# ddlau/modular_rl

Measured on NVIDIA B200. Metric: trpo_update_timesteps_per_sec, higher is better.
Workload: dtype f32

## Files before the change

### modular_rl_b200/csrc/batch_params.cu

```cuda
#include <cstdlib>
#include "common.cuh"
#include "kernels.h"
#include "comm.h"

__global__ void pack_params_kernel(NetGeom g, const float* __restrict__ theta, float* __restrict__ img,
                                   float* __restrict__ WB, int nu) {
  const int i = blockIdx.x * blockDim.x + threadIdx.x;
  const int n_wb = g.d0p * nu;
  if (i < n_wb) {
    const int k = i / nu, n = i % nu;
    const float x = (k < g.d[0] && n < g.d[1]) ? theta[g.off_flat_W[1] + k * g.d[1] + n] : 0.f;
    const float h = tf32_rna(x);
    float* base = WB + (size_t)(k >> 3) * (2 * nu * 8) + ((k & 7) >> 2) * (nu * 4) + (n >> 3) * 32 + (n & 7) * 4 + (k & 3);
    base[0] = h;
    base[nu * 8] = tf32_rna(x - h);
    return;
  }
  const int j = i - n_wb;
  if (j >= g.img_floats) return;
  float v = 0.f;
  if (j < g.bias_floats) {
    if (j >= g.off_pm_logstd) {
      const int q = j - g.off_pm_logstd;
      if (g.off_flat_logstd >= 0 && q < g.d[g.L]) v = theta[g.off_flat_logstd + q];
    } else {
      for (int l = g.L; l >= 1; --l)
        if (j >= g.off_b[l]) {
          const int q = j - g.off_b[l];
          if (q < g.d[l]) v = theta[g.off_flat_b[l] + q];
          break;
        }
    }
  } else if (j < g.bw_floats) {
    for (int l = g.L; l >= 2; --l)
      if (j >= g.off_W[l]) {
        const int q = j - g.off_W[l];
        const int row = q / g.ldw[l], col = q % g.ldw[l];
        if (col < g.d[l]) v = theta[g.off_flat_W[l] + row * g.d[l] + col];
        break;
      }
  } else {
    for (int l = g.L; l >= 2; --l)
      if (j >= g.off_WT[l]) {
        const int q = j - g.off_WT[l];
        const int row = q / g.ldt[l], col = q % g.ldt[l];
        if (col < g.d[l - 1]) v = theta[g.off_flat_W[l] + col * g.d[l] + row];
        break;
      }
  }
  img[j] = v;
}

#define RED_PX 32
#define RED_SY 8
#define RED_UN 8
#define RED_GATHER_CTAS 296
#define RED_GB 5
static_assert(RED_SY >= MRL_P2P_MAX_WORLD, "one thread row per rank in the exchange phase");
__global__ void __launch_bounds__(RED_PX * RED_SY) reduce_partials_kernel(
    NetGeom g, const float* __restrict__ part1, const float* __restrict__ partm, int n_slabs, double scale,
    const float* __restrict__ theta, double l2c2, const float* __restrict__ vlogstd_src, double vls,
    float* __restrict__ out32, double* __restrict__ out64, P2pPush push, P2pGather ga) {
  __shared__ double acc[RED_SY][RED_PX];
  const int px = threadIdx.x, sy = threadIdx.y;
  const int n_chunks = (g.P + RED_PX - 1) / RED_PX;
  for (int chunk = blockIdx.x; chunk < n_chunks; chunk += gridDim.x) {
    const int i = chunk * RED_PX + px;
    double s0 = 0.0, s1 = 0.0;
// ... 275 lines not shown
```

### modular_rl_b200/csrc/common.cuh

```cuda
#pragma once
#include <cuda_runtime.h>
#include <stdint.h>

#define MRL_TILE 64
#define MRL_LDT 68
#define MRL_MAX_LAYERS 6
#define MRL_MID_THREADS 256
#define MRL_MAX_SLAB_TILES 16

enum { MRL_HEAD_GAUSS = 0, MRL_HEAD_CAT = 1, MRL_HEAD_VALUE = 2 };
enum { MRL_ACT_TANH = 0, MRL_ACT_RELU = 1, MRL_ACT_SIGMOID = 2 };
enum { MRL_MODE_GRAD = 0, MRL_MODE_FVP = 1 };

static inline __host__ __device__ int round_up(int x, int m) { return (x + m - 1) / m * m; }

struct NetGeom {
  int L;
  int d[MRL_MAX_LAYERS + 1];
  int head, act;
  int d0p;
  int n1p;
  int ldw[MRL_MAX_LAYERS + 1];
  int ldt[MRL_MAX_LAYERS + 1];
  int off_b[MRL_MAX_LAYERS + 1];
// ... 29 lines not shown
      ".reg .pred p;\n"
      "WAIT_%=:\n"
      "mbarrier.try_wait.parity.shared::cta.b64 p, [%0], %1;\n"
      "@p bra DONE_%=;\n"
      "bra WAIT_%=;\n"
      "DONE_%=:\n"
      "}\n" ::"r"(smem_u32(bar)),
      "r"(parity)
      : "memory");
}
__device__ __forceinline__ void fence_barrier_init() {
  asm volatile("fence.mbarrier_init.release.cluster;" ::: "memory");
}
__device__ __forceinline__ void fence_proxy_async() {
  asm volatile("fence.proxy.async.shared::cta;" ::: "memory");
}
__device__ __forceinline__ void bulk_g2s(void* dst_smem, const void* src_gmem, uint32_t bytes, uint64_t* bar) {
  asm volatile("cp.async.bulk.shared::cluster.global.mbarrier::complete_tx::bytes [%0], [%1], %2, [%3];" ::"r"(
                   smem_u32(dst_smem)),
               "l"(src_gmem), "r"(bytes), "r"(smem_u32(bar))
               : "memory");
}

template <int ACT>
__device__ __forceinline__ float act_fn(float z) {
  if (ACT == MRL_ACT_TANH) return tanhf(z);
  if (ACT == MRL_ACT_RELU) return fmaxf(z, 0.f);
  return 1.f / (1.f + expf(-z));
}
template <int ACT>
__device__ __forceinline__ float dact_from_h(float h) {
  if (ACT == MRL_ACT_TANH) return 1.f - h * h;
  if (ACT == MRL_ACT_RELU) return h > 0.f ? 1.f : 0.f;
  return h * (1.f - h);
}

__device__ __forceinline__ float u_minus_log1p(float u) {
  if (fabsf(u) < 0.2f) {
    float p = 1.f / 12.f;
    p = 1.f / 11.f - u * p; p = 1.f / 10.f - u * p; p = 1.f / 9.f - u * p; p = 1.f / 8.f - u * p;
    p = 1.f / 7.f - u * p;  p = 1.f / 6.f - u * p;  p = 1.f / 5.f - u * p; p = 1.f / 4.f - u * p;
    p = 1.f / 3.f - u * p;  p = 0.5f - u * p;
    return u * u * p;
  }
  return u - log1pf(u);
}

__device__ __forceinline__ float tf32_rna(float x) {
  uint32_t u;
  asm("cvt.rna.tf32.f32 %0, %1;" : "=r"(u) : "f"(x));
  return __uint_as_float(u);
}

__device__ __forceinline__ float warp_sum(float v) {
#pragma unroll
  for (int o = 16; o > 0; o >>= 1) v += __shfl_xor_sync(0xffffffffu, v, o);
  return v;
}
__device__ __forceinline__ double warp_sum(double v) {
#pragma unroll
  for (int o = 16; o > 0; o >>= 1) v += __shfl_xor_sync(0xffffffffu, v, o);
  return v;
}
__device__ __forceinline__ double block_sum(double v, double* scratch) {
  v = warp_sum(v);
  int lane = threadIdx.x & 31, w = threadIdx.x >> 5;
  __syncthreads();
  if (lane == 0) scratch[w] = v;
  __syncthreads();
  int nw = (blockDim.x + 31) >> 5;
  double t = 0.0;
  if (w == 0) {
    t = lane < nw ? scratch[lane] : 0.0;
    t = warp_sum(t);
  }
  return t;
}

void mrl_build_geom(NetGeom* g, int n_layers, const int* dims, int head, int act, int naux);
int mrl_sm_count();
cudaError_t mrl_func_smem(const void* func, size_t bytes);
```

### modular_rl_b200/csrc/geom.cu

```cuda
#include "common.cuh"
#include <string.h>
#include <mutex>
#include <vector>

int mrl_sm_count() {
  static int cache[64] = {0};
  int dev = 0;
  if (cudaGetDevice(&dev) != cudaSuccess || dev < 0 || dev >= 64) return 148;
  if (cache[dev] == 0) {
    int sms = 0;
    if (cudaDeviceGetAttribute(&sms, cudaDevAttrMultiProcessorCount, dev) != cudaSuccess || sms <= 0) sms = 148;
    cache[dev] = sms;
  }
  return cache[dev];
}
cudaError_t mrl_func_smem(const void* func, size_t bytes) {
  struct Ent { const void* f; int dev; size_t bytes; };
  static std::vector<Ent> seen;
  static std::mutex mu;
  int dev = 0;
  cudaError_t e = cudaGetDevice(&dev);
  if (e != cudaSuccess) return e;
  std::lock_guard<std::mutex> lk(mu);
  for (Ent& en : seen)
    if (en.f == func && en.dev == dev) {
      if (bytes <= en.bytes) return cudaSuccess;
      e = cudaFuncSetAttribute(func, cudaFuncAttributeMaxDynamicSharedMemorySize, (int)bytes);
      if (e == cudaSuccess) en.bytes = bytes;
      return e;
    }
  e = cudaFuncSetAttribute(func, cudaFuncAttributeMaxDynamicSharedMemorySize, (int)bytes);
  if (e == cudaSuccess) seen.push_back({func, dev, bytes});
  return e;
}

void mrl_build_geom(NetGeom* g, int n_layers, const int* dims, int head, int act, int naux) {
  memset(g, 0, sizeof(*g));
  g->L = n_layers;
  for (int l = 0; l <= n_layers; ++l) g->d[l] = dims[l];
  g->head = head;
  g->act = act;
  g->d0p = round_up(dims[0], 8);
  g->n1p = round_up(dims[1], 8);
  int pos = 0;
  for (int l = 1; l <= n_layers; ++l) {
    g->off_flat_W[l] = pos;
    pos += dims[l - 1] * dims[l];
    g->off_flat_b[l] = pos;
    pos += dims[l];
  }
  g->off_flat_logstd = -1;
  if (head == MRL_HEAD_GAUSS) {
    g->off_flat_logstd = pos;
    pos += dims[n_layers];
  }
  g->P = pos;
  int off = 0;
  for (int l = 1; l <= n_layers; ++l) {
    g->off_b[l] = off;
    off += round_up(dims[l], 4);
  }
  g->off_pm_logstd = off;
  off += round_up(dims[n_layers], 4);
  g->bias_floats = off;
  for (int l = 2; l <= n_layers; ++l) {
    g->ldw[l] = round_up(dims[l], 4);
    g->off_W[l] = off;
    off += dims[l - 1] * g->ldw[l];
  }
  g->bw_floats = off;
  for (int l = 2; l <= n_layers; ++l) {
    g->ldt[l] = round_up(dims[l - 1], 4);
    g->off_WT[l] = off;
    off += dims[l] * g->ldt[l];
  }
  g->img_floats = off;
  int rows = 0;
  for (int l = 1; l <= n_layers; ++l) {
    g->off_act[l] = rows;
    rows += dims[l];
  }
  g->act_rows = rows;
  g->naux = naux;
  g->pmid = g->bw_floats;
}
```

### modular_rl_b200/csrc/mlp_fvp_tc.cu

```cuda
#include "common.cuh"
#include "kernels.h"
#include "tc_common.cuh"
#include <string.h>

#define FT_THREADS 768
#define FT_RSTAGES 3
#define FT_DSTAGES 3
#define FT_KSLOTS 4
#define FT_MAX_R 3
#define FT_MAX_D 6
#define FT_MAX_PASS 3
#define FT_TMEM_COLS 512

struct FtRStage {
  int l, kgs, N, acc_col, w_off, v_off;
};
struct FtDStage {
  int l, kgs, N, col0, acc_col, w_off;
};
struct FtPlan {
  int L, nR, nD;
  int Kg[MRL_MAX_LAYERS + 1], Np[MRL_MAX_LAYERS + 1];
  int vboff[MRL_MAX_LAYERS + 1];
  FtRStage rs[FT_MAX_R];
// ... 764 lines not shown
                    const float send = (lane & 4) ? val[0] : val[1];
                    const float keep = (lane & 4) ? val[1] : val[0];
                    val[0] = keep + __shfl_xor_sync(0xffffffffu, send, 4);
                  }
                  val[0] += __shfl_xor_sync(0xffffffffu, val[0], 2);
                  val[0] += __shfl_xor_sync(0xffffffffu, val[0], 1);
                  if ((lane & 3) == 0) gb1w[c0 + ((lane >> 4) & 1) * 4 + ((lane >> 3) & 1) * 2 + ((lane >> 2) & 1)] += val[0];
#pragma unroll
                  for (int i = 0; i < 8; ++i) h1c[i] = h1n[i];
                }
                tc_fence_before();
                if (tr_on) FT_TR(4, (8 << 24) | c);
              }
            }
          }
        }
        ft_dbar();
        float* part = a.partm + (size_t)slab * g.pmid;
        const int et = threadIdx.x - 384;
        for (int f = et; f < g.d[1]; f += 256) {
          float sum = 0.f;
#pragma unroll
          for (int w = 0; w < 8; ++w) sum += gb1s[w * 128 + f];
          part[g.off_b[1] + f] = sum;
        }
        for (int j = et; j < g.d[L]; j += 256) part[g.off_pm_logstd + j] = 0.f;
        ft_dbar();
        for (int f = et; f < 8 * 128; f += 256) gb1s[f] = 0.f;
        ft_dbar();
      }
    }
  }
#undef FT_FOR_TILES
  tc_fence_before();
  __syncthreads();
  if (warp == 1) {
    __syncwarp();
    tc_fence_after();
    asm volatile("tcgen05.dealloc.cta_group::1.sync.aligned.b32 %0, %1;" ::"r"(tmem_base), "r"((uint32_t)FT_TMEM_COLS));
  }
}

struct FtPackJob { int off, N, kgs, l, transposed, col0, end; };
struct FtPackJobs { FtPackJob j[FT_MAX_R + FT_MAX_D]; int n; };
__global__ void ft_pack_kernel(NetGeom g, FtPackJobs jobs, const float* __restrict__ src, float* __restrict__ dst, int total,
                               float* __restrict__ WB1, int nu) {
  const int i = blockIdx.x * blockDim.x + threadIdx.x;
  if (i >= total) {
    const int j = i - total;
    if (WB1 == nullptr || j >= g.d0p * nu) return;
    const int k = j / nu, n = j % nu;
    const float x = (k < g.d[0] && n < g.d[1]) ? src[g.off_flat_W[1] + k * g.d[1] + n] : 0.f;
    const float h = tf32_rna(x);
    float* base = WB1 + (size_t)(k >> 3) * (2 * nu * 8) + ((k & 7) >> 2) * (nu * 4) + (n >> 3) * 32 + (n & 7) * 4 + (k & 3);
    base[0] = h;
    base[nu * 8] = tf32_rna(x - h);
    return;
  }
  int q = 0, base = 0;
  while (q < jobs.n - 1 && i >= jobs.j[q].end) { base = jobs.j[q].end; ++q; }
  const FtPackJob jb = jobs.j[q];
  const int e = i - base, K = jb.kgs * 8;
  const int n = e / K, k = e % K;
  const int l = jb.l;
  float x = 0.f;
  if (!jb.transposed) {
    if (n < g.d[l] && k < g.d[l - 1]) x = src[g.off_flat_W[l] + k * g.d[l] + n];
  } else {
    if (n + jb.col0 < g.d[l - 1] && k < g.d[l]) x = src[g.off_flat_W[l] + (n + jb.col0) * g.d[l] + k];
  }
  const float h = tf32_rna(x);
  float* p = dst + jb.off + (size_t)(k >> 3) * (2 * jb.N * 8) + ((k & 7) >> 2) * (jb.N * 4) + (n >> 3) * 32 + (n & 7) * 4 + (k & 3);
  p[0] = h;
  p[jb.N * 8] = tf32_rna(x - h);
}

static bool ft_build_plan(const NetGeom& g, FtPlan* P) {
  memset(P, 0, sizeof(*P));
  const int L = g.L;
  if (L < 3 || L > 4) return false;
  if (g.head != MRL_HEAD_GAUSS && g.head != MRL_HEAD_CAT) return false;
  if (g.d[L] > 64) return false;
  P->L = L;
  int vb = 0;
  for (int l = 1; l <= L; ++l) {
    if (g.d[l] > 128) return false;
    if (l >= 2 && g.d[l] > 64) return false;
    P->Kg[l] = (g.d[l] + 7) / 8;
    P->Np[l] = round_up(g.d[l], 16);
    P->vboff[l] = vb;
    vb += round_up(g.d[l], 16) + 16;
  }
  if (vb > 512) return false;
  if (P->Np[1] != l1tc_nu(g)) return false;
  int wc = 0, vc = 0;
  P->nR = L - 1;
  for (int l = 2; l <= L; ++l) {
    FtRStage& st = P->rs[l - 2];
    st.l = l; st.kgs = P->Kg[l - 1]; st.N = P->Np[l];
    st.w_off = wc; st.v_off = vc;
    wc += st.kgs * 2 * st.N * 8;
    vc += st.kgs * 2 * st.N * 8;
    if (2 * 2 * 2 * st.N * 8 > P->rstage_floats) P->rstage_floats = 2 * 2 * 2 * st.N * 8;
  }
  int nD = 0;
  for (int l = L; l >= 2; --l) {
    P->dstage_of[l] = nD;
    const int Nout = P->Np[l - 1];
    for (int col0 = 0; col0 < Nout; col0 += 64) {
// ... 127 lines not shown
```

### modular_rl_b200/csrc/mlp_l1_tc.cu

```cuda
#include <cstdlib>
#include "common.cuh"
#include "kernels.h"
#include "tc_common.cuh"

#define TC_STAGES 12
#define TC_CGROUPS 2
#define TC_THREADS (192 + 128 * TC_CGROUPS)
#define TC_M 128

#ifdef MRL_TRACE
__device__ long long g_trace[8][512];
#define TRACE(e, u) do { if (blockIdx.x == 0 && (u) < 512) g_trace[e][u] = clock64(); } while (0)
extern "C" int mrl_debug_l1_trace(long long* out) { return cudaMemcpyFromSymbol(out, g_trace, sizeof(g_trace)) != cudaSuccess; }
#else
#define TRACE(e, u) do { } while (0)
#endif
__device__ __forceinline__ void convert_stage(unsigned char* st, int blocks, uint32_t lo_off, int lane) {
  for (int b = 0; b < blocks; ++b) {
    float4* p = reinterpret_cast<float4*>(st + (size_t)b * 4096) + lane;
    float4* pl = reinterpret_cast<float4*>(st + (size_t)b * 4096 + lo_off) + lane;
    float4 x[8];
#pragma unroll
    for (int j = 0; j < 8; ++j) x[j] = p[32 * j];
#pragma unroll
    for (int j = 0; j < 8; ++j) {
      float4 h, l;
#define MRL_SPLIT(X, H, L_)                                                   \
      H = __uint_as_float((__float_as_uint(X) + 0x1000u) & 0xffffe000u);     \
      L_ = __uint_as_float(__float_as_uint(X - H) + 0x1000u);
      MRL_SPLIT(x[j].x, h.x, l.x) MRL_SPLIT(x[j].y, h.y, l.y) MRL_SPLIT(x[j].z, h.z, l.z) MRL_SPLIT(x[j].w, h.w, l.w)
#undef MRL_SPLIT
      p[32 * j] = h;
      pl[32 * j] = l;
    }
  }
  fence_proxy_async();
}

__global__ void __launch_bounds__(TC_THREADS, 1) l1_forward_tc_kernel(const float* __restrict__ XA,
                                                                      const float* __restrict__ WB,
                                                                      float* __restrict__ Zt, int kgroups,
                                                                      int xa_kgroups, int nu, int d1, int n_mtiles,
                                                                      int n_tiles, int acc_cols, int n_acc, int tmem_cols,
                                                                      int nstages, int kps, int cgroups) {
  extern __shared__ __align__(1024) unsigned char smem_raw[];
  uint64_t* full = reinterpret_cast<uint64_t*>(smem_raw);
  uint64_t* empty = full + TC_STAGES;
  uint64_t* tfull = empty + TC_STAGES;
  uint64_t* tempty = tfull + 2;
  uint64_t* conv = tempty + 2;
  uint32_t* tmem_slot = reinterpret_cast<uint32_t*>(conv + TC_STAGES);
  unsigned char* stages = smem_raw + 512;
  const uint32_t blkA = TC_M * 8 * 4, bytesB = 2 * nu * 8 * 4;
  const uint32_t offB = kps * blkA;
  const uint32_t stage_bytes = offB + kps * bytesB;
  const int spt = (kgroups + kps - 1) / kps;
  const uint32_t a_col0 = n_acc * acc_cols;
  const int warp = threadIdx.x >> 5, lane = threadIdx.x & 31;

  if (threadIdx.x == 0) {
    for (int s = 0; s < nstages; ++s) { mbar_init(&full[s], 1); mbar_init(&empty[s], 1); mbar_init(&conv[s], 4); }
    for (int a = 0; a < 2; ++a) { mbar_init(&tfull[a], 1); mbar_init(&tempty[a], 4); }
    fence_barrier_init();
  }
  if (warp == 1) {
    asm volatile("tcgen05.alloc.cta_group::1.sync.aligned.shared::cta.b32 [%0], %1;" ::"r"(smem_u32(tmem_slot)),
                 "r"((uint32_t)tmem_cols));
    asm volatile("tcgen05.relinquish_alloc_permit.cta_group::1.sync.aligned;" ::);
  }
  tc_fence_before();
  __syncthreads();
  tc_fence_after();
  const uint32_t tmem_base = *tmem_slot;

  if (warp == 0) {
    if (lane == 0) {
      int s = 0, ph = 0, u = 0;
      for (int mt = blockIdx.x; mt < n_mtiles; mt += gridDim.x) {
        const float* a_src = XA + (size_t)mt * xa_kgroups * (TC_M * 8);
        for (int q = 0; q < spt; ++q, ++u) {
          const int kg0 = q * kps, nk = min(kps, kgroups - kg0);
          mbar_wait_guard(&empty[s], ph ^ 1);
          TRACE(0, u);
          unsigned char* st = stages + (size_t)s * stage_bytes;
          mbar_expect_tx(&full[s], nk * (blkA + bytesB));
          bulk_g2s(st, a_src + (size_t)kg0 * (TC_M * 8), nk * blkA, &full[s]);
          bulk_g2s(st + offB, WB + (size_t)kg0 * (2 * nu * 8), nk * bytesB, &full[s]);
          TRACE(1, u);
          if (++s == nstages) { s = 0; ph ^= 1; }
        }
      }
    }
  } else if (warp == 1) {
    {
      const uint32_t idesc = (1u << 4) | (2u << 7) | (2u << 10) | ((uint32_t)(nu >> 3) << 17) | ((TC_M >> 4) << 24);
      const uint32_t lboB = nu * 4 * 4;
      const uint32_t desc_hi = (uint32_t)(umma_desc(0, 0, 128) >> 32);
      const uint32_t dB0 = umma_desc_lo(smem_u32(stages) + offB, lboB);
      uint32_t tcount = 0;
      int s = 0, ph = 0, u = 0;
      bool next_ready = false;
      for (int mt = blockIdx.x; mt < n_mtiles; mt += gridDim.x, ++tcount) {
        const int acc = n_acc == 2 ? (tcount & 1) : 0;
        mbar_wait_guard(&tempty[acc], (n_acc == 2 ? ((tcount >> 1) & 1) : (tcount & 1)) ^ 1);
        tc_fence_after();
        const uint32_t d_tmem = tmem_base + acc * acc_cols;
        for (int q = 0; q < spt; ++q, ++u) {
          const int nk = min(kps, kgroups - q * kps);
          TRACE(4, u);
          if (!next_ready) mbar_wait_guard(&conv[s], ph);
          TRACE(6, u);
          tc_fence_after();
          uint32_t db = dB0 + s * (stage_bytes >> 4);
          uint32_t ta = tmem_base + a_col0 + (uint32_t)(s * kps) * 16;
          if (elect_one()) {
            for (int j = 0; j < nk; ++j) {
              umma_tf32_ts(d_tmem, ta + 8, db, desc_hi, idesc, (q | j) ? 1u : 0u);
              umma_tf32_ts(d_tmem, ta, db + (bytesB >> 5), desc_hi, idesc, 1u);
              umma_tf32_ts(d_tmem, ta, db, desc_hi, idesc, 1u);
              ta += 16;
              db += bytesB >> 4;
            }
            tc_commit(&empty[s]);
            if (q == spt - 1) tc_commit(&tfull[acc]);
          }
          __syncwarp();
          {
            const int sn = s + 1 == nstages ? 0 : s + 1;
            next_ready = mbar_probe(&conv[sn], s + 1 == nstages ? ph ^ 1 : ph);
          }
          TRACE(7, u);
          if (++s == nstages) { s = 0; ph ^= 1; }
        }
      }
    }
  } else if (warp >= 6) {
    const int quarter = warp & 3;
    const int m = quarter * 32 + lane;
    const int cgroup = (warp - 6) >> 2;
    int s = cgroup, ph = 0, u = 0;
    for (int mt = blockIdx.x; cgroup < cgroups && mt < n_mtiles; mt += gridDim.x) {
      for (int q = 0; q < spt; ++q, ++u) {
        if ((u & (cgroups - 1)) != cgroup) continue;
        const int nk = min(kps, kgroups - q * kps);
        mbar_wait_guard(&full[s], ph);
        if (warp == 6 && lane == 0) TRACE(2, u);
        const unsigned char* st = stages + (size_t)s * stage_bytes;
        uint32_t ta = tmem_base + ((uint32_t)(quarter * 32) << 16) + a_col0 + (uint32_t)(s * kps) * 16;
        for (int j = 0; j < nk; ++j) {
          const float4 x0 = *reinterpret_cast<const float4*>(st + (size_t)j * blkA + (size_t)m * 16);
          const float4 x1 = *reinterpret_cast<const float4*>(st + (size_t)j * blkA + 2048 + (size_t)m * 16);
          const float x[8] = {x0.x, x0.y, x0.z, x0.w, x1.x, x1.y, x1.z, x1.w};
          uint32_t hi[8], lo[8];
#pragma unroll
          for (int k = 0; k < 8; ++k) {
            hi[k] = (__float_as_uint(x[k]) + 0x1000u) & 0xffffe000u;
            lo[k] = __float_as_uint(x[k] - __uint_as_float(hi[k])) + 0x1000u;
          }
          tmem_st8(ta, hi);
          tmem_st8(ta + 8, lo);
          ta += 16;
        }
        asm volatile("tcgen05.wait::st.sync.aligned;" ::: "memory");
        tc_fence_before();
        __syncwarp();
        if (lane == 0) mbar_arrive(&conv[s]);
        if (warp == 6 && lane == 0) TRACE(3, u);
        s += cgroups;
        if (s >= nstages) { s -= nstages; ph ^= 1; }
      }
    }
  } else if (warp >= 2 && warp < 6) {
    const int q = warp & 3;
    uint32_t tcount = 0;
    for (int mt = blockIdx.x; mt < n_mtiles; mt += gridDim.x, ++tcount) {
      const int acc = n_acc == 2 ? (tcount & 1) : 0;
      mbar_wait_guard(&tfull[acc], n_acc == 2 ? ((tcount >> 1) & 1) : (tcount & 1));
      tc_fence_after();
      const int r = q * 32 + lane;
      const int tile = 2 * mt + (r >> 6);
      float* zt = Zt + ((size_t)tile * d1) * MRL_LDT + (r & 63);
      const uint32_t taddr = tmem_base + ((uint32_t)(q * 32) << 16) + acc * acc_cols;
      for (int c0 = 0; c0 < nu; c0 += 16) {
        uint32_t v[16];
        tmem_ld16(taddr + c0, v);
        if (tile < n_tiles) {
#pragma unroll
          for (int j = 0; j < 16; ++j)
            if (c0 + j < d1) zt[(size_t)(c0 + j) * MRL_LDT] = __uint_as_float(v[j]);
        }
      }
      tc_fence_before();
      __syncwarp();
      if (lane == 0) mbar_arrive(&tempty[acc]);
    }
  }
  tc_fence_before();
  __syncthreads();
  if (warp == 1) {
    __syncwarp();
    tc_fence_after();
    asm volatile("tcgen05.dealloc.cta_group::1.sync.aligned.b32 %0, %1;" ::"r"(tmem_base), "r"((uint32_t)tmem_cols));
  }
}

__global__ void __launch_bounds__(TC_THREADS, 1) l1_grad_tc_kernel(const float* __restrict__ XG,
                                                                   const float* __restrict__ DG,
                                                                   float* __restrict__ part1, int ftiles,
                                                                   int xg_ftiles, int nu, int d0, int n1p,
                                                                   int slab_tiles, int n_tiles, int n_slabs,
                                                                   int acc_stride, int tmem_cols, int nss, int nts,
                                                                   int dg_mn, int cgroups) {
  extern __shared__ __align__(1024) unsigned char smem_raw[];
  uint64_t* full = reinterpret_cast<uint64_t*>(smem_raw);
  uint64_t* sempty = full + TC_STAGES;
  uint64_t* conv = sempty + TC_STAGES;
  uint64_t* aempty = conv + TC_STAGES;
  uint64_t* tfull = aempty + TC_STAGES;
  uint64_t* tempty = tfull + 1;
  uint32_t* tmem_slot = reinterpret_cast<uint32_t*>(tempty + 1);
  unsigned char* stages = smem_raw + 512;
  const uint32_t blkA = TC_M * 8 * 4, bytesB = 2 * nu * 8 * 4;
  const uint32_t offB = ftiles * blkA;
  const uint32_t stage_bytes = offB + bytesB;
  const uint32_t a_col0 = ftiles * acc_stride;
  const int warp = threadIdx.x >> 5, lane = threadIdx.x & 31;

  if (threadIdx.x == 0) {
    for (int s = 0; s < nss; ++s) { mbar_init(&full[s], 1); mbar_init(&sempty[s], 1); }
    for (int s = 0; s < nts; ++s) { mbar_init(&conv[s], 4); mbar_init(&aempty[s], 1); }
    mbar_init(&tfull[0], 1);
    mbar_init(&tempty[0], 4);
    fence_barrier_init();
  }
  if (warp == 1) {
    asm volatile("tcgen05.alloc.cta_group::1.sync.aligned.shared::cta.b32 [%0], %1;" ::"r"(smem_u32(tmem_slot)),
                 "r"((uint32_t)tmem_cols));
    asm volatile("tcgen05.relinquish_alloc_permit.cta_group::1.sync.aligned;" ::);
  }
  tc_fence_before();
  __syncthreads();
  tc_fence_after();
  const uint32_t tmem_base = *tmem_slot;

  if (warp == 0) {
    if (lane == 0) {
      int s = 0, ph = 0;
      for (int slab = blockIdx.x; slab < n_slabs; slab += gridDim.x) {
        const int t0 = slab * slab_tiles, t1 = min(t0 + slab_tiles, n_tiles);
        for (int tg = t0 * 8; tg < t1 * 8; ++tg) {
          mbar_wait_guard(&sempty[s], ph ^ 1);
          unsigned char* st = stages + (size_t)s * stage_bytes;
          mbar_expect_tx(&full[s], offB + bytesB);
          bulk_g2s(st, XG + (size_t)tg * xg_ftiles * (TC_M * 8), offB, &full[s]);
          bulk_g2s(st + offB, DG + (size_t)tg * (2 * nu * 8), bytesB, &full[s]);
// ... 107 lines not shown
    asm volatile("tcgen05.dealloc.cta_group::1.sync.aligned.b32 %0, %1;" ::"r"(tmem_base), "r"((uint32_t)tmem_cols));
  }
}

template <typename T>
__global__ void pack_xa_kernel(const T* __restrict__ src, long long ld, int ncols, long long N, float* __restrict__ XA,
                               int xa_kgroups, long long rows_out) {
  const long long i = (long long)blockIdx.x * blockDim.x + threadIdx.x;
  const int quads = xa_kgroups * 2;
  if (i >= rows_out * quads) return;
  const long long t = i / quads;
  const int kq4 = (int)(i % quads);
  const int kg = kq4 >> 1, khalf = kq4 & 1;
  const long long mt = t / TC_M;
  const int m = (int)(t % TC_M);
  float x[4];
#pragma unroll
  for (int j = 0; j < 4; ++j) {
    const int c = 4 * kq4 + j;
    x[j] = (t < N && c < ncols) ? (float)src[t * ld + c] : 0.f;
  }
  float* base = XA + ((size_t)mt * xa_kgroups + kg) * (TC_M * 8) + khalf * (TC_M * 4) + (m >> 3) * 32 + (m & 7) * 4;
  *reinterpret_cast<float4*>(base) = make_float4(x[0], x[1], x[2], x[3]);
}
template <typename T>
__global__ void pack_xg_kernel(const T* __restrict__ src, long long ld, int ncols, long long N, float* __restrict__ XG,
                               int xg_ftiles, long long n_tquads) {
  const int fpad = xg_ftiles * TC_M;
  const long long i = (long long)blockIdx.x * blockDim.x + threadIdx.x;
  if (i >= n_tquads * fpad) return;
  const long long tq = i / fpad;
  const int f = (int)(i % fpad);
  float x[4];
#pragma unroll
  for (int j = 0; j < 4; ++j) {
    const long long t = tq * 4 + j;
    x[j] = (t < N && f < ncols) ? (float)src[t * ld + f] : 0.f;
  }
  const long long tg = tq >> 1;
  const int khalf = (int)(tq & 1), ft = f / TC_M, fm = f % TC_M;
  float* base = XG + ((size_t)tg * xg_ftiles + ft) * (TC_M * 8) + khalf * (TC_M * 4) + (fm >> 3) * 32 + (fm & 7) * 4;
  *reinterpret_cast<float4*>(base) = make_float4(x[0], x[1], x[2], x[3]);
}

int l1tc_nu(const NetGeom& g) { return round_up(g.d[1], 16); }
size_t l1tc_wb_floats(const NetGeom& g) { return (size_t)g.d0p * l1tc_nu(g) * 2; }
size_t l1tc_xa_floats(int xa_kgroups, long long n_mtiles) { return (size_t)n_mtiles * xa_kgroups * TC_M * 8; }

cudaError_t launch_l1_forward_tc(const NetGeom& g, const float* XA, int xa_kgroups, const float* WB, float* Zt,
                                 int n_tiles, cudaStream_t st) {
  const int nu = l1tc_nu(g);
  const int acc_cols = nu <= 32 ? 32 : (nu <= 64 ? 64 : (nu <= 128 ? 128 : 256));
  const int n_acc = acc_cols <= 128 ? 2 : 1;
  static const int kps_env = getenv("MRL_L1_KPS") ? atoi(getenv("MRL_L1_KPS")) : 0;
  static const int cg_env = getenv("MRL_L1_CGROUPS") ? atoi(getenv("MRL_L1_CGROUPS")) : 0;
  int kps = 0, nstages = 0, cgroups = 1;
  for (int pass = 0; pass < 2; ++pass) {
    kps = kps_env > 0 ? kps_env : (pass == 0 ? 4 : 3);
    const size_t sb = (size_t)kps * (TC_M * 8 * 4 + 2 * (size_t)nu * 8 * 4);
    nstages = (int)((227 * 1024 - 512) / sb);
    const int tmem_room = (512 - n_acc * acc_cols) / (kps * 16);
    if (nstages > tmem_room) nstages = tmem_room;
    if (nstages > TC_STAGES) nstages = TC_STAGES;
    cgroups = (pass == 0 && nstages >= 4) ? 2 : 1;
    if (cg_env > 0) cgroups = (cg_env >= 2 && nstages >= 2) ? 2 : 1;
    if (cgroups == 2) nstages &= ~1;
    if (cgroups == 2 || cg_env > 0 || kps_env > 0) break;
  }
  if (nstages < 2) return cudaErrorInvalidConfiguration;
  const size_t stage_bytes = (size_t)kps * (TC_M * 8 * 4 + 2 * (size_t)nu * 8 * 4);
  int tmem_cols = 32;
  while (tmem_cols < n_acc * acc_cols + nstages * kps * 16) tmem_cols *= 2;
  const size_t smem = 512 + (size_t)nstages * stage_bytes;
  {
    cudaError_t e = mrl_func_smem((const void*)l1_forward_tc_kernel, smem);
    if (e != cudaSuccess) return e;
  }
  const int sms = mrl_sm_count();
  const int n_mtiles = (n_tiles + 1) / 2;
  const int grid = n_mtiles < sms ? n_mtiles : sms;
  l1_forward_tc_kernel<<<grid, TC_THREADS, smem, st>>>(XA, WB, Zt, g.d0p / 8, xa_kgroups, nu, g.d[1], n_mtiles, n_tiles,
                                                       acc_cols, n_acc, tmem_cols, nstages, kps, cgroups);
  return cudaGetLastError();
}

cudaError_t launch_pack_xa(const void* src, int dtype, long long ld, int ncols, long long N, float* XA, int xa_kgroups,
                           long long n_mtiles, cudaStream_t st) {
  const long long rows_out = n_mtiles * TC_M;
  const long long total = rows_out * xa_kgroups * 2;
  const unsigned blocks = (unsigned)((total + 255) / 256);
  if (dtype == 1) pack_xa_kernel<double><<<blocks, 256, 0, st>>>((const double*)src, ld, ncols, N, XA, xa_kgroups, rows_out);
  else pack_xa_kernel<float><<<blocks, 256, 0, st>>>((const float*)src, ld, ncols, N, XA, xa_kgroups, rows_out);
  return cudaGetLastError();
}
size_t l1tc_xg_floats(int xg_ftiles, long long n_tiles) { return (size_t)n_tiles * 8 * xg_ftiles * TC_M * 8; }
size_t l1tc_dg_floats(const NetGeom& g, long long n_tiles) { return (size_t)n_tiles * 8 * 2 * l1tc_nu(g) * 8; }

cudaError_t launch_pack_xg(const void* src, int dtype, long long ld, int ncols, long long N, float* XG, int xg_ftiles,
                           long long n_tiles, cudaStream_t st) {
  const long long n_tquads = n_tiles * 16;
  const long long total = n_tquads * xg_ftiles * TC_M;
  const unsigned blocks = (unsigned)((total + 255) / 256);
  if (dtype == 1) pack_xg_kernel<double><<<blocks, 256, 0, st>>>((const double*)src, ld, ncols, N, XG, xg_ftiles, n_tquads);
  else pack_xg_kernel<float><<<blocks, 256, 0, st>>>((const float*)src, ld, ncols, N, XG, xg_ftiles, n_tquads);
  return cudaGetLastError();
}

static bool l1g_plan(const NetGeom& g, int* acc_stride, int* nts, int* nss, int* tmem_cols, size_t* smem) {
  const int nu = l1tc_nu(g);
  const int ftiles = (g.d[0] + TC_M - 1) / TC_M;
  *acc_stride = nu;
  *nts = (512 - ftiles * nu) / (ftiles * 16);
  if (*nts > TC_STAGES) *nts = TC_STAGES;
  const size_t stage_bytes = (size_t)ftiles * TC_M * 8 * 4 + 2 * (size_t)nu * 8 * 4;
  *nss = (int)((227 * 1024 - 512) / stage_bytes);
  if (*nss > TC_STAGES) *nss = TC_STAGES;
  *tmem_cols = 32;
  while (*tmem_cols < ftiles * nu + *nts * ftiles * 16) *tmem_cols *= 2;
  *smem = 512 + (size_t)*nss * stage_bytes;
  return nu <= 256 && *nts >= 1 && *nss >= 2 && *tmem_cols <= 512;
}

cudaError_t launch_l1_grad_tc(const NetGeom& g, const float* XG, int xg_ftiles, const float* DG, float* part1,
                              int slab_tiles, int n_tiles, int n_slabs, cudaStream_t st, int dg_mn_major) {
  const int nu = l1tc_nu(g);
  const int ftiles = (g.d[0] + TC_M - 1) / TC_M;
  int acc_stride, nts, nss, tmem_cols;
  size_t smem;
  if (!l1g_plan(g, &acc_stride, &nts, &nss, &tmem_cols, &smem)) return cudaErrorInvalidConfiguration;
  {
    cudaError_t e = mrl_func_smem((const void*)l1_grad_tc_kernel, smem);
    if (e != cudaSuccess) return e;
  }
  static const int cg_env = getenv("MRL_L1_CGROUPS") ? atoi(getenv("MRL_L1_CGROUPS")) : 0;
  int cgroups = (nts >= 2 && nss >= 4) ? 2 : 1;
// ... 15 lines not shown
```

### modular_rl_b200/csrc/tc_common.cuh

```cuda
#pragma once
#include "common.cuh"

#define TC_WATCHDOG (1u << 27)
__device__ __forceinline__ void mbar_wait_guard(uint64_t* bar, uint32_t parity) {
  uint32_t done = 0, spins = 0;
  while (true) {
    asm volatile(
        "{\n.reg .pred p;\n"
        "mbarrier.try_wait.parity.shared::cta.b64 p, [%1], %2;\n"
        "selp.u32 %0, 1, 0, p;\n}\n"
        : "=r"(done)
        : "r"(smem_u32(bar)), "r"(parity)
        : "memory");
    if (done) return;
    if (++spins > TC_WATCHDOG) __trap();
  }
}
template <int NS>
__device__ __forceinline__ void mbar_wait_ns(uint64_t* bar, uint32_t parity) {
  uint32_t done = 0, spins = 0;
  while (true) {
    asm volatile(
        "{\n.reg .pred p;\n"
        "mbarrier.try_wait.parity.shared::cta.b64 p, [%1], %2;\n"
        "selp.u32 %0, 1, 0, p;\n}\n"
        : "=r"(done)
        : "r"(smem_u32(bar)), "r"(parity)
        : "memory");
    if (done) return;
    __nanosleep(NS);
    if (++spins > (1u << 24)) __trap();
  }
}
#ifndef MRL_WAIT_NS
#define MRL_WAIT_NS 40
#endif
__device__ __forceinline__ void mbar_wait_sleep(uint64_t* bar, uint32_t parity) { mbar_wait_ns<MRL_WAIT_NS>(bar, parity); }
__device__ __forceinline__ bool elect_one() {
  uint32_t pred;
  asm volatile("{\n.reg .pred P;\nelect.sync _|P, 0xffffffff;\nselp.u32 %0, 1, 0, P;\n}\n" : "=r"(pred));
  return pred != 0;
}
__device__ __forceinline__ bool mbar_probe(uint64_t* bar, uint32_t parity) {
  uint32_t done;
  asm volatile(
      "{\n.reg .pred p;\n"
      "mbarrier.test_wait.parity.shared::cta.b64 p, [%1], %2;\n"
      "selp.u32 %0, 1, 0, p;\n}\n"
      : "=r"(done)
      : "r"(smem_u32(bar)), "r"(parity)
      : "memory");
  return done != 0;
}
__device__ __forceinline__ void mbar_arrive(uint64_t* bar) {
  asm volatile("mbarrier.arrive.shared::cta.b64 _, [%0];" ::"r"(smem_u32(bar)) : "memory");
}
__device__ __forceinline__ void tc_fence_before() { asm volatile("tcgen05.fence::before_thread_sync;" ::: "memory"); }
__device__ __forceinline__ void tc_fence_after() { asm volatile("tcgen05.fence::after_thread_sync;" ::: "memory"); }
__device__ __forceinline__ void tc_commit(uint64_t* bar) {
  asm volatile("tcgen05.commit.cta_group::1.mbarrier::arrive::one.shared::cluster.b64 [%0];" ::"r"(smem_u32(bar))
               : "memory");
}
__device__ __forceinline__ uint64_t umma_desc(uint32_t smem_addr, uint32_t lbo_bytes, uint32_t sbo_bytes) {
  return (uint64_t)((smem_addr >> 4) & 0x3FFF) | ((uint64_t)((lbo_bytes >> 4) & 0x3FFF) << 16) |
         ((uint64_t)((sbo_bytes >> 4) & 0x3FFF) << 32) | (1ull << 46);
}
__device__ __forceinline__ uint32_t umma_desc_lo(uint32_t smem_addr, uint32_t lbo_bytes) {
  return ((smem_addr >> 4) & 0x3FFF) | (((lbo_bytes >> 4) & 0x3FFF) << 16);
}
__device__ __forceinline__ void umma_tf32_lo(uint32_t tmem_d, uint32_t da_lo, uint32_t db_lo, uint32_t desc_hi,
                                             uint32_t idesc, uint32_t acc) {
  asm volatile(
      "{\n.reg .pred p;\n.reg .b64 da, db;\n"
      "setp.ne.b32 p, %5, 0;\n"
      "mov.b64 da, {%1, %3};\n"
      "mov.b64 db, {%2, %3};\n"
      "tcgen05.mma.cta_group::1.kind::tf32 [%0], da, db, %4, p;\n}\n" ::"r"(tmem_d),
      "r"(da_lo), "r"(db_lo), "r"(desc_hi), "r"(idesc), "r"(acc)
      : "memory");
}
__device__ __forceinline__ void umma_tf32_ts(uint32_t tmem_d, uint32_t tmem_a, uint32_t db_lo, uint32_t desc_hi,
                                             uint32_t idesc, uint32_t acc) {
  asm volatile(
      "{\n.reg .pred p;\n.reg .b64 db;\n"
      "setp.ne.b32 p, %5, 0;\n"
      "mov.b64 db, {%2, %3};\n"
      "tcgen05.mma.cta_group::1.kind::tf32 [%0], [%1], db, %4, p;\n}\n" ::"r"(tmem_d),
      "r"(tmem_a), "r"(db_lo), "r"(desc_hi), "r"(idesc), "r"(acc)
      : "memory");
}
__device__ __forceinline__ void tmem_st8(uint32_t taddr, const uint32_t (&r)[8]) {
  asm volatile("tcgen05.st.sync.aligned.32x32b.x8.b32 [%0], {%1, %2, %3, %4, %5, %6, %7, %8};\n" ::"r"(taddr), "r"(r[0]),
               "r"(r[1]), "r"(r[2]), "r"(r[3]), "r"(r[4]), "r"(r[5]), "r"(r[6]), "r"(r[7])
               : "memory");
}
__device__ __forceinline__ void umma_tf32(uint32_t tmem_d, uint64_t da, uint64_t db, uint32_t idesc, uint32_t acc) {
  asm volatile(
      "{\n.reg .pred p;\n"
      "setp.ne.b32 p, %4, 0;\n"
      "tcgen05.mma.cta_group::1.kind::tf32 [%0], %1, %2, %3, p;\n}\n" ::"r"(tmem_d),
      "l"(da), "l"(db), "r"(idesc), "r"(acc)
      : "memory");
}
__device__ __forceinline__ void tmem_ld16(uint32_t taddr, uint32_t (&r)[16]) {
  asm volatile(
      "tcgen05.ld.sync.aligned.32x32b.x16.b32 {%0, %1, %2, %3, %4, %5, %6, %7, %8, %9, %10, %11, %12, %13, %14, %15}, "
      "[%16];\n"
      : "=r"(r[0]), "=r"(r[1]), "=r"(r[2]), "=r"(r[3]), "=r"(r[4]), "=r"(r[5]), "=r"(r[6]), "=r"(r[7]), "=r"(r[8]),
        "=r"(r[9]), "=r"(r[10]), "=r"(r[11]), "=r"(r[12]), "=r"(r[13]), "=r"(r[14]), "=r"(r[15])
// ... 5 lines not shown
```

Measured before the change: 34.59 million.

## Convert layer-1 tensor-core forward to 2-CTA cluster MMA with split B operand

Moves the layer-1 forward GEMM from single-CTA tcgen05 MMA to cta_group::2 pair MMA, with M=256 split across a 2-CTA cluster. Each CTA now loads only half of the hi/lo weight B operand, and the WB packing layout is changed to store those halves separately. The smem stage ring and the TMEM A-operand ring are split into independent pipelines with their own barriers, and converter/epilogue warps signal the leader CTA through cluster-mapped mbarriers. This reduces per-CTA B traffic and smem footprint to allow deeper pipelining, at the cost of cluster synchronisation, a fixed kps and the removal of the environment tuning knobs.

```diff
diff --git a/modular_rl_b200/csrc/batch_params.cu b/modular_rl_b200/csrc/batch_params.cu
--- a/modular_rl_b200/csrc/batch_params.cu
+++ b/modular_rl_b200/csrc/batch_params.cu
@@ -11,9 +11,9 @@
     const int k = i / nu, n = i % nu;
     const float x = (k < g.d[0] && n < g.d[1]) ? theta[g.off_flat_W[1] + k * g.d[1] + n] : 0.f;
     const float h = tf32_rna(x);
-    float* base = WB + (size_t)(k >> 3) * (2 * nu * 8) + ((k & 7) >> 2) * (nu * 4) + (n >> 3) * 32 + (n & 7) * 4 + (k & 3);
+    float* base = WB + l1tc_wb_offset(k, n, nu, g.d0p);
     base[0] = h;
-    base[nu * 8] = tf32_rna(x - h);
+    base[nu * 4] = tf32_rna(x - h);
     return;
   }
   const int j = i - n_wb;
diff --git a/modular_rl_b200/csrc/common.cuh b/modular_rl_b200/csrc/common.cuh
--- a/modular_rl_b200/csrc/common.cuh
+++ b/modular_rl_b200/csrc/common.cuh
@@ -105,6 +105,12 @@
   return __uint_as_float(u);
 }
 
+__device__ __forceinline__ size_t l1tc_wb_offset(int k, int n, int nu, int d0p) {
+  const int h = n >= (nu >> 1), nn = n - h * (nu >> 1);
+  return (size_t)h * d0p * nu + (size_t)(k >> 3) * (nu * 8) + ((k & 7) >> 2) * (nu * 2) + (nn >> 3) * 32 + (nn & 7) * 4 +
+         (k & 3);
+}
+
 __device__ __forceinline__ float warp_sum(float v) {
 #pragma unroll
   for (int o = 16; o > 0; o >>= 1) v += __shfl_xor_sync(0xffffffffu, v, o);
@@ -133,3 +139,4 @@
 void mrl_build_geom(NetGeom* g, int n_layers, const int* dims, int head, int act, int naux);
 int mrl_sm_count();
 cudaError_t mrl_func_smem(const void* func, size_t bytes);
+cudaError_t mrl_max_clusters(const void* func, int threads, size_t smem, int* clusters);
diff --git a/modular_rl_b200/csrc/geom.cu b/modular_rl_b200/csrc/geom.cu
--- a/modular_rl_b200/csrc/geom.cu
+++ b/modular_rl_b200/csrc/geom.cu
@@ -32,6 +32,29 @@
   e = cudaFuncSetAttribute(func, cudaFuncAttributeMaxDynamicSharedMemorySize, (int)bytes);
   if (e == cudaSuccess) seen.push_back({func, dev, bytes});
   return e;
+}
+
+cudaError_t mrl_max_clusters(const void* func, int threads, size_t smem, int* clusters) {
+  struct Ent { const void* f; int dev; size_t smem; int n; };
+  static std::vector<Ent> seen;
+  static std::mutex mu;
+  int dev = 0;
+  cudaError_t e = cudaGetDevice(&dev);
+  if (e != cudaSuccess) return e;
+  std::lock_guard<std::mutex> lk(mu);
+  for (const Ent& en : seen)
+    if (en.f == func && en.dev == dev && en.smem == smem) { *clusters = en.n; return cudaSuccess; }
+  cudaLaunchConfig_t cfg = {};
+  cfg.gridDim = dim3(2 * mrl_sm_count(), 1, 1);
+  cfg.blockDim = dim3(threads, 1, 1);
+  cfg.dynamicSmemBytes = smem;
+  int n = 0;
+  e = cudaOccupancyMaxActiveClusters(&n, func, &cfg);
+  if (e != cudaSuccess) return e;
+  if (n < 1) return cudaErrorInvalidConfiguration;
+  seen.push_back({func, dev, smem, n});
+  *clusters = n;
+  return cudaSuccess;
 }
 
 void mrl_build_geom(NetGeom* g, int n_layers, const int* dims, int head, int act, int naux) {
diff --git a/modular_rl_b200/csrc/mlp_fvp_tc.cu b/modular_rl_b200/csrc/mlp_fvp_tc.cu
--- a/modular_rl_b200/csrc/mlp_fvp_tc.cu
+++ b/modular_rl_b200/csrc/mlp_fvp_tc.cu
@@ -840,9 +840,9 @@
     const int k = j / nu, n = j % nu;
     const float x = (k < g.d[0] && n < g.d[1]) ? src[g.off_flat_W[1] + k * g.d[1] + n] : 0.f;
     const float h = tf32_rna(x);
-    float* base = WB1 + (size_t)(k >> 3) * (2 * nu * 8) + ((k & 7) >> 2) * (nu * 4) + (n >> 3) * 32 + (n & 7) * 4 + (k & 3);
+    float* base = WB1 + l1tc_wb_offset(k, n, nu, g.d0p);
     base[0] = h;
-    base[nu * 8] = tf32_rna(x - h);
+    base[nu * 4] = tf32_rna(x - h);
     return;
   }
   int q = 0, base = 0;
diff --git a/modular_rl_b200/csrc/mlp_l1_tc.cu b/modular_rl_b200/csrc/mlp_l1_tc.cu
--- a/modular_rl_b200/csrc/mlp_l1_tc.cu
+++ b/modular_rl_b200/csrc/mlp_l1_tc.cu
@@ -37,70 +37,76 @@
   fence_proxy_async();
 }
 
-__global__ void __launch_bounds__(TC_THREADS, 1) l1_forward_tc_kernel(const float* __restrict__ XA,
-                                                                      const float* __restrict__ WB,
-                                                                      float* __restrict__ Zt, int kgroups,
-                                                                      int xa_kgroups, int nu, int d1, int n_mtiles,
-                                                                      int n_tiles, int acc_cols, int n_acc, int tmem_cols,
-                                                                      int nstages, int kps, int cgroups) {
+__global__ void __cluster_dims__(2, 1, 1) __launch_bounds__(TC_THREADS, 1)
+    l1_forward_tc_kernel(const float* __restrict__ XA, const float* __restrict__ WB, float* __restrict__ Zt, int kgroups,
+                         int xa_kgroups, int nu, int d1, int n_mtiles, int n_tiles, int acc_cols, int n_acc,
+                         int tmem_cols, int nss, int nts, int kps, int cgroups) {
   extern __shared__ __align__(1024) unsigned char smem_raw[];
   uint64_t* full = reinterpret_cast<uint64_t*>(smem_raw);
-  uint64_t* empty = full + TC_STAGES;
-  uint64_t* tfull = empty + TC_STAGES;
+  uint64_t* sempty = full + TC_STAGES;
+  uint64_t* aempty = sempty + TC_STAGES;
+  uint64_t* conv = aempty + TC_STAGES;
+  uint64_t* tfull = conv + TC_STAGES;
   uint64_t* tempty = tfull + 2;
-  uint64_t* conv = tempty + 2;
-  uint32_t* tmem_slot = reinterpret_cast<uint32_t*>(conv + TC_STAGES);
+  uint32_t* tmem_slot = reinterpret_cast<uint32_t*>(tempty + 2);
   unsigned char* stages = smem_raw + 512;
-  const uint32_t blkA = TC_M * 8 * 4, bytesB = 2 * nu * 8 * 4;
+  const uint32_t blkA = TC_M * 8 * 4, bytesB = nu * 8 * 4;
   const uint32_t offB = kps * blkA;
   const uint32_t stage_bytes = offB + kps * bytesB;
   const int spt = (kgroups + kps - 1) / kps;
   const uint32_t a_col0 = n_acc * acc_cols;
   const int warp = threadIdx.x >> 5, lane = threadIdx.x & 31;
+  const uint32_t rank = cluster_ctarank();
+  const int pair = blockIdx.x >> 1, npairs = gridDim.x >> 1;
+  const int n_ptiles = (n_mtiles + 1) >> 1;
 
   if (threadIdx.x == 0) {
-    for (int s = 0; s < nstages; ++s) { mbar_init(&full[s], 1); mbar_init(&empty[s], 1); mbar_init(&conv[s], 4); }
-    for (int a = 0; a < 2; ++a) { mbar_init(&tfull[a], 1); mbar_init(&tempty[a], 4); }
+    for (int s = 0; s < nss; ++s) { mbar_init(&full[s], 1); mbar_init(&sempty[s], 1); }
+    for (int a = 0; a < nts; ++a) { mbar_init(&aempty[a], 1); mbar_init(&conv[a], 8); }
+    for (int a = 0; a < 2; ++a) { mbar_init(&tfull[a], 1); mbar_init(&tempty[a], 8); }
     fence_barrier_init();
   }
   if (warp == 1) {
-    asm volatile("tcgen05.alloc.cta_group::1.sync.aligned.shared::cta.b32 [%0], %1;" ::"r"(smem_u32(tmem_slot)),
+    asm volatile("tcgen05.alloc.cta_group::2.sync.aligned.shared::cta.b32 [%0], %1;" ::"r"(smem_u32(tmem_slot)),
                  "r"((uint32_t)tmem_cols));
-    asm volatile("tcgen05.relinquish_alloc_permit.cta_group::1.sync.aligned;" ::);
+    asm volatile("tcgen05.relinquish_alloc_permit.cta_group::2.sync.aligned;" ::);
   }
   tc_fence_before();
-  __syncthreads();
+  cluster_sync();
   tc_fence_after();
   const uint32_t tmem_base = *tmem_slot;
 
   if (warp == 0) {
     if (lane == 0) {
       int s = 0, ph = 0, u = 0;
-      for (int mt = blockIdx.x; mt < n_mtiles; mt += gridDim.x) {
+      const float* b_src = WB + (size_t)rank * kgroups * (nu * 8);
+      for (int pt = pair; pt < n_ptiles; pt += npairs) {
+        const int mt = 2 * pt + (int)rank;
+        const bool has_a = mt < n_mtiles;
         const float* a_src = XA + (size_t)mt * xa_kgroups * (TC_M * 8);
         for (int q = 0; q < spt; ++q, ++u) {
           const int kg0 = q * kps, nk = min(kps, kgroups - kg0);
-          mbar_wait_guard(&empty[s], ph ^ 1);
+          mbar_wait_guard(&sempty[s], ph ^ 1);
           TRACE(0, u);
           unsigned char* st = stages + (size_t)s * stage_bytes;
-          mbar_expect_tx(&full[s], nk * (blkA + bytesB));
-          bulk_g2s(st, a_src + (size_t)kg0 * (TC_M * 8), nk * blkA, &full[s]);
-          bulk_g2s(st + offB, WB + (size_t)kg0 * (2 * nu * 8), nk * bytesB, &full[s]);
+          mbar_expect_tx(&full[s], nk * ((has_a ? blkA : 0u) + bytesB));
+          if (has_a) bulk_g2s(st, a_src + (size_t)kg0 * (TC_M * 8), nk * blkA, &full[s]);
+          bulk_g2s(st + offB, b_src + (size_t)kg0 * (nu * 8), nk * bytesB, &full[s]);
           TRACE(1, u);
-          if (++s == nstages) { s = 0; ph ^= 1; }
+          if (++s == nss) { s = 0; ph ^= 1; }
         }
       }
     }
   } else if (warp == 1) {
-    {
-      const uint32_t idesc = (1u << 4) | (2u << 7) | (2u << 10) | ((uint32_t)(nu >> 3) << 17) | ((TC_M >> 4) << 24);
-      const uint32_t lboB = nu * 4 * 4;
+    if (rank == 0) {
+      const uint32_t idesc = (1u << 4) | (2u << 7) | (2u << 10) | ((uint32_t)(nu >> 3) << 17) | ((2 * TC_M >> 4) << 24);
+      const uint32_t lboB = nu * 8;
       const uint32_t desc_hi = (uint32_t)(umma_desc(0, 0, 128) >> 32);
       const uint32_t dB0 = umma_desc_lo(smem_u32(stages) + offB, lboB);
       uint32_t tcount = 0;
-      int s = 0, ph = 0, u = 0;
+      int s = 0, a = 0, aph = 0, u = 0;
       bool next_ready = false;
-      for (int mt = blockIdx.x; mt < n_mtiles; mt += gridDim.x, ++tcount) {
+      for (int pt = pair; pt < n_ptiles; pt += npairs, ++tcount) {
         const int acc = n_acc == 2 ? (tcount & 1) : 0;
         mbar_wait_guard(&tempty[acc], (n_acc == 2 ? ((tcount >> 1) & 1) : (tcount & 1)) ^ 1);
         tc_fence_after();
@@ -108,29 +114,31 @@
         for (int q = 0; q < spt; ++q, ++u) {
           const int nk = min(kps, kgroups - q * kps);
           TRACE(4, u);
-          if (!next_ready) mbar_wait_guard(&conv[s], ph);
+          if (!next_ready) mbar_wait_guard(&conv[a], aph);
           TRACE(6, u);
           tc_fence_after();
           uint32_t db = dB0 + s * (stage_bytes >> 4);
-          uint32_t ta = tmem_base + a_col0 + (uint32_t)(s * kps) * 16;
+          uint32_t ta = tmem_base + a_col0 + (uint32_t)(a * kps) * 16;
           if (elect_one()) {
             for (int j = 0; j < nk; ++j) {
-              umma_tf32_ts(d_tmem, ta + 8, db, desc_hi, idesc, (q | j) ? 1u : 0u);
-              umma_tf32_ts(d_tmem, ta, db + (bytesB >> 5), desc_hi, idesc, 1u);
-              umma_tf32_ts(d_tmem, ta, db, desc_hi, idesc, 1u);
+              umma_tf32_ts_pair(d_tmem, ta + 8, db, desc_hi, idesc, (q | j) ? 1u : 0u);
+              umma_tf32_ts_pair(d_tmem, ta, db + (bytesB >> 5), desc_hi, idesc, 1u);
+              umma_tf32_ts_pair(d_tmem, ta, db, desc_hi, idesc, 1u);
               ta += 16;
               db += bytesB >> 4;
             }
-            tc_commit(&empty[s]);
-            if (q == spt - 1) tc_commit(&tfull[acc]);
+            tc_commit_pair(&sempty[s]);
+            tc_commit_pair(&aempty[a]);
+            if (q == spt - 1) tc_commit_pair(&tfull[acc]);
           }
           __syncwarp();
           {
-            const int sn = s + 1 == nstages ? 0 : s + 1;
-            next_ready = mbar_probe(&conv[sn], s + 1 == nstages ? ph ^ 1 : ph);
+            const int an = a + 1 == nts ? 0 : a + 1;
+            next_ready = mbar_probe(&conv[an], a + 1 == nts ? aph ^ 1 : aph);
           }
           TRACE(7, u);
-          if (++s == nstages) { s = 0; ph ^= 1; }
+          if (++s == nss) s = 0;
+          if (++a == nts) { a = 0; aph ^= 1; }
         }
       }
     }
@@ -138,16 +146,19 @@
     const int quarter = warp & 3;
     const int m = quarter * 32 + lane;
     const int cgroup = (warp - 6) >> 2;
-    int s = cgroup, ph = 0, u = 0;
-    for (int mt = blockIdx.x; cgroup < cgroups && mt < n_mtiles; mt += gridDim.x) {
+    int s = cgroup, ph = 0, a = cgroup, aph = 0, u = 0;
+    for (int pt = pair; cgroup < cgroups && pt < n_ptiles; pt += npairs) {
+      const bool has_a = 2 * pt + (int)rank < n_mtiles;
       for (int q = 0; q < spt; ++q, ++u) {
         if ((u & (cgroups - 1)) != cgroup) continue;
         const int nk = min(kps, kgroups - q * kps);
         mbar_wait_guard(&full[s], ph);
+        mbar_wait_guard(&aempty[a], aph ^ 1);
+        tc_fence_after();
         if (warp == 6 && lane == 0) TRACE(2, u);
         const unsigned char* st = stages + (size_t)s * stage_bytes;
-        uint32_t ta = tmem_base + ((uint32_t)(quarter * 32) << 16) + a_col0 + (uint32_t)(s * kps) * 16;
-        for (int j = 0; j < nk; ++j) {
+        uint32_t ta = tmem_base + ((uint32_t)(quarter * 32) << 16) + a_col0 + (uint32_t)(a * kps) * 16;
+        for (int j = 0; has_a && j < nk; ++j) {
           const float4 x0 = *reinterpret_cast<const float4*>(st + (size_t)j * blkA + (size_t)m * 16);
           const float4 x1 = *reinterpret_cast<const float4*>(st + (size_t)j * blkA + 2048 + (size_t)m * 16);
           const float x[8] = {x0.x, x0.y, x0.z, x0.w, x1.x, x1.y, x1.z, x1.w};
@@ -164,21 +175,23 @@
         asm volatile("tcgen05.wait::st.sync.aligned;" ::: "memory");
         tc_fence_before();
         __syncwarp();
-        if (lane == 0) mbar_arrive(&conv[s]);
+        if (lane == 0) mbar_arrive_cluster(&conv[a], 0);
         if (warp == 6 && lane == 0) TRACE(3, u);
         s += cgroups;
-        if (s >= nstages) { s -= nstages; ph ^= 1; }
+        if (s >= nss) { s -= nss; ph ^= 1; }
+        a += cgroups;
+        if (a >= nts) { a -= nts; aph ^= 1; }
       }
     }
   } else if (warp >= 2 && warp < 6) {
     const int q = warp & 3;
     uint32_t tcount = 0;
-    for (int mt = blockIdx.x; mt < n_mtiles; mt += gridDim.x, ++tcount) {
+    for (int pt = pair; pt < n_ptiles; pt += npairs, ++tcount) {
       const int acc = n_acc == 2 ? (tcount & 1) : 0;
       mbar_wait_guard(&tfull[acc], n_acc == 2 ? ((tcount >> 1) & 1) : (tcount & 1));
       tc_fence_after();
       const int r = q * 32 + lane;
-      const int tile = 2 * mt + (r >> 6);
+      const int tile = 2 * (2 * pt + (int)rank) + (r >> 6);
       float* zt = Zt + ((size_t)tile * d1) * MRL_LDT + (r & 63);
       const uint32_t taddr = tmem_base + ((uint32_t)(q * 32) << 16) + acc * acc_cols;
       for (int c0 = 0; c0 < nu; c0 += 16) {
@@ -192,15 +205,15 @@
       }
       tc_fence_before();
       __syncwarp();
-      if (lane == 0) mbar_arrive(&tempty[acc]);
+      if (lane == 0) mbar_arrive_cluster(&tempty[acc], 0);
     }
   }
   tc_fence_before();
-  __syncthreads();
+  cluster_sync();
   if (warp == 1) {
     __syncwarp();
     tc_fence_after();
-    asm volatile("tcgen05.dealloc.cta_group::1.sync.aligned.b32 %0, %1;" ::"r"(tmem_base), "r"((uint32_t)tmem_cols));
+    asm volatile("tcgen05.dealloc.cta_group::2.sync.aligned.b32 %0, %1;" ::"r"(tmem_base), "r"((uint32_t)tmem_cols));
   }
 }
 
@@ -414,35 +427,32 @@
   const int nu = l1tc_nu(g);
   const int acc_cols = nu <= 32 ? 32 : (nu <= 64 ? 64 : (nu <= 128 ? 128 : 256));
   const int n_acc = acc_cols <= 128 ? 2 : 1;
-  static const int kps_env = getenv("MRL_L1_KPS") ? atoi(getenv("MRL_L1_KPS")) : 0;
-  static const int cg_env = getenv("MRL_L1_CGROUPS") ? atoi(getenv("MRL_L1_CGROUPS")) : 0;
-  int kps = 0, nstages = 0, cgroups = 1;
-  for (int pass = 0; pass < 2; ++pass) {
-    kps = kps_env > 0 ? kps_env : (pass == 0 ? 4 : 3);
-    const size_t sb = (size_t)kps * (TC_M * 8 * 4 + 2 * (size_t)nu * 8 * 4);
-    nstages = (int)((227 * 1024 - 512) / sb);
-    const int tmem_room = (512 - n_acc * acc_cols) / (kps * 16);
-    if (nstages > tmem_room) nstages = tmem_room;
-    if (nstages > TC_STAGES) nstages = TC_STAGES;
-    cgroups = (pass == 0 && nstages >= 4) ? 2 : 1;
-    if (cg_env > 0) cgroups = (cg_env >= 2 && nstages >= 2) ? 2 : 1;
-    if (cgroups == 2) nstages &= ~1;
-    if (cgroups == 2 || cg_env > 0 || kps_env > 0) break;
-  }
-  if (nstages < 2) return cudaErrorInvalidConfiguration;
-  const size_t stage_bytes = (size_t)kps * (TC_M * 8 * 4 + 2 * (size_t)nu * 8 * 4);
+  const int kps = 4;
+  const size_t stage_bytes = (size_t)kps * (TC_M * 8 * 4 + (size_t)nu * 8 * 4);
+  int nss = (int)((227 * 1024 - 512) / stage_bytes);
+  int nts = (512 - n_acc * acc_cols) / (kps * 16);
+  if (nss > TC_STAGES) nss = TC_STAGES;
+  if (nts > TC_STAGES) nts = TC_STAGES;
+  const int cgroups = (nts >= 2 && nss >= 2) ? 2 : 1;
+  if (cgroups == 2) { nss &= ~1; nts &= ~1; }
+  if (nss < 2 || nts < 1) return cudaErrorInvalidConfiguration;
   int tmem_cols = 32;
-  while (tmem_cols < n_acc * acc_cols + nstages * kps * 16) tmem_cols *= 2;
-  const size_t smem = 512 + (size_t)nstages * stage_bytes;
+  while (tmem_cols < n_acc * acc_cols + nts * kps * 16) tmem_cols *= 2;
+  const size_t smem = 512 + (size_t)nss * stage_bytes;
   {
     cudaError_t e = mrl_func_smem((const void*)l1_forward_tc_kernel, smem);
     if (e != cudaSuccess) return e;
   }
-  const int sms = mrl_sm_count();
+  int clusters = 0;
+  {
+    cudaError_t e = mrl_max_clusters((const void*)l1_forward_tc_kernel, TC_THREADS, smem, &clusters);
+    if (e != cudaSuccess) return e;
+  }
   const int n_mtiles = (n_tiles + 1) / 2;
-  const int grid = n_mtiles < sms ? n_mtiles : sms;
-  l1_forward_tc_kernel<<<grid, TC_THREADS, smem, st>>>(XA, WB, Zt, g.d0p / 8, xa_kgroups, nu, g.d[1], n_mtiles, n_tiles,
-                                                       acc_cols, n_acc, tmem_cols, nstages, kps, cgroups);
+  const int n_ptiles = (n_mtiles + 1) / 2;
+  const int pairs = n_ptiles < clusters ? n_ptiles : clusters;
+  l1_forward_tc_kernel<<<2 * pairs, TC_THREADS, smem, st>>>(XA, WB, Zt, g.d0p / 8, xa_kgroups, nu, g.d[1], n_mtiles,
+                                                            n_tiles, acc_cols, n_acc, tmem_cols, nss, nts, kps, cgroups);
   return cudaGetLastError();
 }
 
diff --git a/modular_rl_b200/csrc/tc_common.cuh b/modular_rl_b200/csrc/tc_common.cuh
--- a/modular_rl_b200/csrc/tc_common.cuh
+++ b/modular_rl_b200/csrc/tc_common.cuh
@@ -55,6 +55,35 @@
 __device__ __forceinline__ void mbar_arrive(uint64_t* bar) {
   asm volatile("mbarrier.arrive.shared::cta.b64 _, [%0];" ::"r"(smem_u32(bar)) : "memory");
 }
+__device__ __forceinline__ uint32_t cluster_ctarank() {
+  uint32_t r;
+  asm volatile("mov.u32 %0, %%cluster_ctarank;" : "=r"(r));
+  return r;
+}
+__device__ __forceinline__ void cluster_sync() {
+  asm volatile("barrier.cluster.arrive.release.aligned;\nbarrier.cluster.wait.acquire.aligned;" ::: "memory");
+}
+__device__ __forceinline__ void mbar_arrive_cluster(uint64_t* bar, uint32_t rank) {
+  uint32_t raddr;
+  asm volatile("mapa.shared::cluster.u32 %0, %1, %2;" : "=r"(raddr) : "r"(smem_u32(bar)), "r"(rank));
+  asm volatile("mbarrier.arrive.shared::cluster.b64 _, [%0];" ::"r"(raddr) : "memory");
+}
+__device__ __forceinline__ void tc_commit_pair(uint64_t* bar) {
+  asm volatile("tcgen05.commit.cta_group::2.mbarrier::arrive::one.shared::cluster.multicast::cluster.b64 [%0], %1;" ::"r"(
+                   smem_u32(bar)),
+               "h"((uint16_t)3)
+               : "memory");
+}
+__device__ __forceinline__ void umma_tf32_ts_pair(uint32_t tmem_d, uint32_t tmem_a, uint32_t db_lo, uint32_t desc_hi,
+                                                  uint32_t idesc, uint32_t acc) {
+  asm volatile(
+      "{\n.reg .pred p;\n.reg .b64 db;\n"
+      "setp.ne.b32 p, %5, 0;\n"
+      "mov.b64 db, {%2, %3};\n"
+      "tcgen05.mma.cta_group::2.kind::tf32 [%0], [%1], db, %4, p;\n}\n" ::"r"(tmem_d),
+      "r"(tmem_a), "r"(db_lo), "r"(desc_hi), "r"(idesc), "r"(acc)
+      : "memory");
+}
 __device__ __forceinline__ void tc_fence_before() { asm volatile("tcgen05.fence::before_thread_sync;" ::: "memory"); }
 __device__ __forceinline__ void tc_fence_after() { asm volatile("tcgen05.fence::after_thread_sync;" ::: "memory"); }
 __device__ __forceinline__ void tc_commit(uint64_t* bar) {
```

After: 35.60 million, median of 6. 1.03x the previous value.
